# FJingxian/JanusX

Hardware: AMD Instinct MI355X
Metric: SNPs/sec full -lmm (GRM+eig+scan) (higher is better)
Workload: dtype f64 (eigendecomposition, REML and per-SNP statistics; GRM and rotation products are exact int8 / split-f16 MFMA sums merged in f64)

## Files before the change

janusx_amd/csrc/eigh.cpp:

```cpp
#include <rocblas/rocblas.h>
#include <rocsolver/rocsolver.h>

#include <stdio.h>
#include <stdlib.h>
#include <string.h>

#include <chrono>
#include <memory>
#include <mutex>
#include <vector>

#include "jx_common.h"

namespace jx {
int launch_add_diag(double *d_a, int n, int64_t ld, double ridge, hipStream_t st);
int launch_symmetrize(double *d_a, int n, hipStream_t st);
int sytrd_lower(rocblas_handle h, hipStream_t st, double *d_a, int n, double *d_d, double *d_e, double *d_tau);
int stedc_split(rocblas_handle h, hipStream_t st, int n, double *d_d, double *d_e, double *d_c, int leaf,
                std::vector<int> &h_perm, int sel_lo = 0, int sel_hi = 0);
int launch_gather_cols(const double *src, const int *d_perm, int n, double *dst, hipStream_t st);
void gather_cols_grid(int n, unsigned *gx, unsigned *gy);
int sytrd_set_dist(int rank, int world, int (*allreduce)(void *), void *user, double *staging, int64_t staging_doubles,
                   int min_n);
int ormtr_lower(hipStream_t st, const double *d_a, int n, const double *d_tau, double *d_c);
size_t sy2sb_work_doubles(int n);
int sy2sb_bandwidth();
int sy2sb_lower(hipStream_t st, double *d_a, int n, double *d_tau, double *d_ab, int ldab, double *d_work, int *d_flags,
                bool allow_shard = false);
int sy2sb_set_band_dist(int rank, int world, int (*allreduce)(void *, int64_t), void *user, double *staging,
                        int64_t staging_doubles, int min_n, int block);
int64_t sy2sb_band_staging_doubles(int n);
int sy2sb_band_dist_active(int n);
int sb2st_ldab();
int sb2st_steps(int n);
size_t sb2st_ctrl_bytes(int n);
int sb2st_chase(hipStream_t st, double *d_ab, int n, double *d_d, double *d_e, double *d_v2, double *d_tau2, int *d_ctrl);
size_t sbback_tq_doubles(int n, int ks);
int sbback_apply_q2(hipStream_t st, const double *d_v2, const double *d_tau2, int n, int ks, double *d_c, int ncols,
                    double *d_tq, hipEvent_t ev_start, hipEvent_t ev_stop);
extern float g_last_ms[24];
int ormtr_lower_off(hipStream_t st, const double *d_a, int n, int off, int nref, const double *d_tau, double *d_c, int ncols);
struct OrmtrPlan;
OrmtrPlan *ormtr_plan_new();
void ormtr_plan_free(OrmtrPlan *p);
int ormtr_prepare(hipStream_t st, const double *d_a, int n, int off, int nref, const double *d_tau, OrmtrPlan &plan);
int ormtr_apply(hipStream_t st, const OrmtrPlan &plan, double *d_c, int ncols);
int sytrd_dist_active(int n);
void sytrd_dist_rank(int *rank, int *world);
void sytrd_dist_pause(int on);
int launch_gather_cols_range(const double *src, const int *d_perm, int n, int count, double *dst, hipStream_t st);
struct EighGather {
    int (*gather)(void *) = nullptr;
    void *user = nullptr;
    int (*agree)(void *, uint64_t) = nullptr;
    void *agree_user = nullptr;
};
static EighGather g_gather;
constexpr int kRocsolverStedcMaxN = 46340;

static rocblas_handle g_handle = nullptr;
static std::mutex g_handle_mu;

static rocblas_handle get_handle() {
    std::lock_guard<std::mutex> lk(g_handle_mu);
    if (!g_handle) {
        if (rocblas_create_handle(&g_handle) != rocblas_status_success) g_handle = nullptr;
        if (g_handle) rocblas_set_atomics_mode(g_handle, rocblas_atomics_not_allowed);
    }
    return g_handle;
}
}

using namespace jx;

extern "C" int64_t jxg_eigh_dist_staging_doubles(int n) { return (int64_t)n + 32 * 16 + 2 * 64; }

// ... 108 lines not shown
        auto flag_on_any_rank = [&](int local_flag, int *any) -> int {
            *any = local_flag != 0;
            if (!dist_two) return 0;
            if (!g_gather.agree) {
                if (local_flag != 0)
                    return fail("jxg_eigh_f64: a reduction stage failed on this rank and no agreement callback is registered "
                                "(jxg_eigh_set_agree): the ranks cannot take the fallback together");
                return 0;
            }
            const int ag = g_gather.agree(g_gather.agree_user, local_flag != 0 ? 0x9e3779b97f4a7c15ull : 0ull);
            if (ag < 0) return fail("jxg_eigh_f64: the agreement callback failed");
            if (ag == 0) *any = 1;
            return 0;
        };
        std::unique_ptr<OrmtrPlan, void (*)(OrmtrPlan *)> q1_plan(nullptr, ormtr_plan_free);
        DevBuf ts_work, ts_ab, ts_tau2, ts_ctrl, ts_flags, ts_tq;
        ScratchLease ts_v2;
        const int ldab = sb2st_ldab(), ks = sb2st_steps(n);
        if (twostage) {
            if (ts_work.alloc(sizeof(double) * sy2sb_work_doubles(n))) return 1;
            if (ts_ab.alloc(sizeof(double) * (size_t)ldab * n)) return 1;
            if (ts_v2.take(4, sizeof(double) * (size_t)n * n)) return 1;
            if (ts_tau2.alloc(sizeof(double) * (size_t)n * ks)) return 1;
            if (ts_ctrl.alloc(sb2st_ctrl_bytes(n))) return 1;
            if (ts_flags.alloc(sizeof(int) * 4)) return 1;
            JX_HIP(hipMemcpyAsync(c.p, d_a, sizeof(double) * (size_t)n * n, hipMemcpyDeviceToDevice, st));
            static const bool force_single = getenv("JXGPU_DIST_EIGH_FORCE") && atoi(getenv("JXGPU_DIST_EIGH_FORCE")) != 0;
            const bool shard_band = (dist_two || force_single) && sy2sb_band_dist_active(n);
            g_last_band_sharded = shard_band ? 1 : 0;
            if (sy2sb_lower(st, d_a, n, tau.as<double>(), ts_ab.as<double>(), ldab, ts_work.as<double>(),
                            ts_flags.as<int>(), shard_band))
                return 1;
            int hf[4] = {0, 0, 0, 0};
            JX_HIP(hipMemcpyAsync(hf, ts_flags.p, sizeof(hf), hipMemcpyDeviceToHost, st));
            {
                size_t fr = 0, tot = 0;
                const size_t need = sizeof(double) * sbback_tq_doubles(n, ks);
                if (hipMemGetInfo(&fr, &tot) == hipSuccess && fr > need + ((size_t)8 << 30) && ts_tq.alloc(need)) return 1;
            }
            JX_HIP(hipStreamSynchronize(st));
            int flagged = 0;
            if (flag_on_any_rank(hf[0], &flagged)) return 1;
            if (flagged) {
                if (trace) (void)stage_done("sy2sb (flagged)");
                if (trace) fprintf(stderr, "[jxgpu eigh n=%d] band reduction flagged a panel (code %d): one-stage fallback\n", n, hf[0]);
                JX_HIP(hipMemcpyAsync(d_a, c.p, sizeof(double) * (size_t)n * n, hipMemcpyDeviceToDevice, st));
                ts_tq.release();
                twostage = false;
            }
        }
        if (twostage) {
            JX_HIP(hipEventRecord(ev[1], st));
            if (stage_done("sy2sb")) return 1;
            if (sb2st_chase(st, ts_ab.as<double>(), n, d_w, e.as<double>(), ts_v2.as<double>(), ts_tau2.as<double>(),
                            ts_ctrl.as<int>()))
                return 1;
            int habort = 0;
            JX_HIP(hipMemcpyAsync(&habort, ts_ctrl.as<int>() + n, sizeof(int), hipMemcpyDeviceToHost, st));
            JX_HIP(hipStreamSynchronize(st));
            int aborted = 0;
            if (flag_on_any_rank(habort, &aborted)) return 1;
            if (aborted) {
                if (trace) fprintf(stderr, "[jxgpu eigh n=%d] bulge chasing gave up waiting for a neighbour sweep: one-stage fallback\n", n);
                JX_HIP(hipMemcpyAsync(d_a, c.p, sizeof(double) * (size_t)n * n, hipMemcpyDeviceToDevice, st));
                ts_tq.release();
                twostage = false;
            } else {
                JX_HIP(hipEventRecord(ev[2], st));
                if (stage_done("sb2st")) return 1;
            }
        }
        if (twostage) q1_plan.reset(ormtr_plan_new());
        if (!twostage) {
            if (sytrd_lower(h, st, d_a, n, d_w, e.as<double>(), tau.as<double>())) return 1;
            if (stage_done("sytrd")) return 1;
        }
        const char *sm = getenv("JXGPU_STEDC");
        bool split = n >= 2048;
        if (sm && strcmp(sm, "rocsolver") == 0 && n <= kRocsolverStedcMaxN) split = false;
        if (sm && strcmp(sm, "split") == 0 && n >= 64) split = true;
        int leaf = getenv("JXGPU_STEDC_LEAF") ? atoi(getenv("JXGPU_STEDC_LEAF")) : 1280;
        if (leaf < 2) leaf = 2;
        if (leaf > kRocsolverStedcMaxN) leaf = kRocsolverStedcMaxN;
        std::vector<int> perm;
        rocblas_status rs = rocblas_status_success;
        bool replicas_agree = true;
        g_last_dist_agree = -1;
// ... 184 lines not shown
```

janusx_amd/csrc/k_dgemm.hip:

```cpp
#include <stdlib.h>

#include "jx_common.h"

namespace jx {

typedef double d4 __attribute__((ext_vector_type(4)));

constexpr int DG_BK = 16;
constexpr int DG_THREADS = 512;

struct DgemmArgs {
    const double *a;
    const double *b;
    double *c;
    int64_t lda, ldb, ldc;
    int m, n, k;
    double alpha, beta;
    int ta, tb;
    int symm_a;
    int lower_tiles;
    int ksplit;
    double *ws;
};

// ... 415 lines not shown
}

static int dg_reduce(hipStream_t st, const DgemmArgs &g) {
    if ((int64_t)g.m * g.n > 0xffffff00LL) return fail("dgemm: result beyond 2^32 elements (one dispatch dimension)");
    const int64_t mn = (int64_t)g.m * g.n;
    if (mn <= 16384 && g.ksplit >= 16)
        hipLaunchKernelGGL(dg_reduce_kernel<8>, dim3((unsigned)((mn + 31) / 32)), dim3(256), 0, st, g.c, g.ldc, g.m, g.n, g.beta, g.ws,
                           g.ksplit);
    else
        hipLaunchKernelGGL(dg_reduce_kernel<1>, dim3((unsigned)((mn + 255) / 256)), dim3(256), 0, st, g.c, g.ldc, g.m, g.n, g.beta, g.ws,
                           g.ksplit);
    JX_LAUNCH_CHECK();
    return 0;
}

int dgemm(hipStream_t st, bool ta, bool tb, int m, int n, int k, double alpha, const double *a, int64_t lda,
          const double *b, int64_t ldb, double beta, double *c, int64_t ldc, int ksplit, double *ws, size_t ws_doubles) {
    if (m <= 0 || n <= 0) return 0;
    DgemmArgs g{a, b, c, lda, ldb, ldc, m, n, k, alpha, beta, ta ? 1 : 0, tb ? 1 : 0, 0, 0, 1, ws};
    if (k <= 0) {
        hipLaunchKernelGGL(dg_scale_kernel, dim3((unsigned)(((int64_t)m * n + 255) / 256)), dim3(256), 0, st, c, ldc, m, n, beta);
        JX_LAUNCH_CHECK();
        return 0;
    }
    const bool small_n = n <= 64, small_m = m <= 64;
    const int bm = small_m ? 64 : 128, bn = (small_n || small_m) ? 64 : 128;
    const int tm = ceil_div(m, bm), tn = ceil_div(n, bn);
    if (ksplit <= 0) {
        const int64_t tiles = (int64_t)tm * tn;
        const int ktiles = ceil_div(k, DG_BK);
        ksplit = 1;
        if (tiles < 384) {
            ksplit = (int)((768 + tiles - 1) / tiles);
            const int maxsplit = ktiles / 8 > 0 ? ktiles / 8 : 1;
            if (ksplit > maxsplit) ksplit = maxsplit;
            if (ksplit < 1) ksplit = 1;
        }
    }
    g.ksplit = dg_fit_split(ksplit, m, n, ws ? ws_doubles : 0);
    dim3 grid(tm, tn, g.ksplit);
    int rc;
    if (bm == 128 && bn == 128) rc = dg_launch<128, 128>(g, grid, st);
    else if (bm == 128) rc = dg_launch<128, 64>(g, grid, st);
    else rc = dg_launch<64, 64>(g, grid, st);
    if (rc) return rc;
    return g.ksplit > 1 ? dg_reduce(st, g) : 0;
}

int dsymm_lower(hipStream_t st, int m, int n, double alpha, const double *a, int64_t lda, const double *b, int64_t ldb,
                double beta, double *c, int64_t ldc, double *ws, size_t ws_doubles) {
    if (m <= 0 || n <= 0) return 0;
    DgemmArgs g{a, b, c, lda, ldb, ldc, m, n, m, alpha, beta, 0, 0, 1, 0, 1, ws};
    const bool wide = n > 64;
// ... 98 lines not shown
```

janusx_amd/csrc/k_ormtr.hip:

```cpp
#include <stdlib.h>

#include <algorithm>
#include <chrono>
#include <vector>

#include "k_ozgemm.h"

namespace jx {

int dgemm(hipStream_t st, bool ta, bool tb, int m, int n, int k, double alpha, const double *a, int64_t lda, const double *b,
          int64_t ldb, double beta, double *c, int64_t ldc, int ksplit, double *ws, size_t ws_doubles);

constexpr int OT_NB = 1024;
constexpr int OT_TB = 64;

__global__ __launch_bounds__(256) void ot_extract_v_kernel(const double *__restrict__ a, int n, int jb, int nbk,
                                                          const double *__restrict__ tau, double *__restrict__ vc,
                                                          int rows, int off) {
    const int k = blockIdx.y;
    const int r = blockIdx.x * 256 + threadIdx.x;
    if (k >= nbk || r >= rows) return;
    const int j = jb + k;
    const int row = jb + off + r;
    double v = 0.0;
    if (tau[j] != 0.0) {
        if (row == j + off) v = 1.0;
        else if (row > j + off) v = a[(int64_t)j * n + row];
    }
    vc[(int64_t)k * rows + r] = v;
}

__global__ void ot_fix_m_kernel(double *__restrict__ m, int nbk, int nb, const double *__restrict__ tau, int jb) {
    const int c = blockIdx.x * blockDim.x + threadIdx.x;
    const int r = blockIdx.y;
    if (c >= nb || r >= nb) return;
    double *p = m + (int64_t)c * nb + r;
    if (r >= nbk || c >= nbk) *p = (r == c) ? 1.0 : 0.0;
    else if (r > c) *p = 0.0;
    else if (r == c) {
        const double t = tau[jb + c];
        *p = (t != 0.0) ? 1.0 / t : 1.0;
    }
}

__global__ __launch_bounds__(OT_TB) void ot_triinv_diag_kernel(const double *__restrict__ m, double *__restrict__ t, int ld) {
    __shared__ double s[OT_TB][OT_TB + 1];
    const int o = blockIdx.x * OT_TB, c = threadIdx.x;
    for (int j = 0; j < OT_TB; ++j) s[c][j] = m[(int64_t)(o + j) * ld + o + c];
    __syncthreads();
    double x[OT_TB];
#pragma unroll
    for (int i = OT_TB - 1; i >= 0; --i) {
        double acc = (i == c) ? 1.0 : 0.0;
#pragma unroll
        for (int k = i + 1; k < OT_TB; ++k) acc -= s[i][k] * x[k];
        x[i] = (i <= c) ? acc / s[i][i] : 0.0;
// ... 21 lines not shown

static int ot_round_nb(int nb) {
    int r = OT_TB;
    while (r * 2 <= nb) r *= 2;
    return r;
}

int ormtr_oz_min_n() {
    static const int v = getenv("JXGPU_OZ_MIN_N") ? atoi(getenv("JXGPU_OZ_MIN_N")) : 3000;
    return v;
}

struct OrmtrBlock {
    int jb = 0, nbk = 0, rows = 0;
    size_t o_vt = 0, o_vtt = 0;
};
struct OrmtrPlan {
    int n = 0, off = 0, nref = 0, nb = 0;
    bool use_oz = false;
    std::vector<OrmtrBlock> blocks;
    ScratchLease work;
    ScratchLease store;
};

OrmtrPlan *ormtr_plan_new() { return new OrmtrPlan(); }
void ormtr_plan_free(OrmtrPlan *p) { delete p; }

int ormtr_prepare(hipStream_t st, const double *d_a, int n, int off, int nref, const double *d_tau, OrmtrPlan &P) {
    P.n = n;
    P.off = off;
    P.nref = nref;
    P.blocks.clear();
    if (n < 2 || nref < 1) return 0;
    static const bool oz_on = !(getenv("JXGPU_ORMTR_OZ") && atoi(getenv("JXGPU_ORMTR_OZ")) == 0);
    P.use_oz = oz_on && n >= ormtr_oz_min_n();
    int nb = (getenv("JXGPU_ORMTR_NB") && atoi(getenv("JXGPU_ORMTR_NB")) > 0) ? atoi(getenv("JXGPU_ORMTR_NB"))
                                                                              : (n >= 12000 ? 2 * OT_NB : OT_NB);
    nb = ot_round_nb(std::max(nb, OT_TB));
    while (nb > OT_TB && nb / 2 >= nref) nb /= 2;
    P.nb = nb;
    const int nblocks = (nref + nb - 1) / nb;
    size_t store_bytes = 0;
    for (int b = nblocks - 1; b >= 0; --b) {
        OrmtrBlock k;
        k.jb = b * nb;
        k.nbk = (nref - k.jb < nb) ? (nref - k.jb) : nb;
        k.rows = n - k.jb - off;
        k.o_vt = store_bytes;
        store_bytes += P.use_oz ? oz_image_bytes(k.nbk, k.rows) : ((sizeof(double) * (size_t)k.rows * k.nbk + 255) & ~(size_t)255);
        k.o_vtt = store_bytes;
        store_bytes += P.use_oz ? oz_image_bytes(k.rows, k.nbk) : ((sizeof(double) * (size_t)k.rows * k.nbk + 255) & ~(size_t)255);
        P.blocks.push_back(k);
    }
    const size_t nvc = (size_t)n * nb, nmm = (size_t)nb * nb;
    const size_t ngws = std::max<size_t>(4 * nmm, (size_t)1 << 20);
    if (P.work.take(3, sizeof(double) * (2 * nvc + 2 * nmm + nmm / 4 + ngws))) return 1;
    if (P.store.take(5, store_bytes + 256)) return 1;
    double *const vc = P.work.as<double>(), *const vt = vc + nvc, *const mm = vt + nvc, *const tt = mm + nmm;
    double *const xw = tt + nmm, *const gws = xw + nmm / 4;
    char *const store = P.store.as<char>();
    for (const OrmtrBlock &k : P.blocks) {
        double *vcb = P.use_oz ? vc : reinterpret_cast<double *>(store + k.o_vt);
        double *vtb = P.use_oz ? vt : reinterpret_cast<double *>(store + k.o_vtt);
        hipLaunchKernelGGL(ot_extract_v_kernel, dim3((k.rows + 255) / 256, k.nbk), dim3(256), 0, st, d_a, n, k.jb, k.nbk, d_tau,
                           vcb, k.rows, off);
        JX_LAUNCH_CHECK();
        if (P.use_oz) {
            OzImage i_vt = oz_image_at(store + k.o_vt, k.nbk, k.rows);
            if (oz_slice(st, vcb, k.rows, 1, i_vt)) return 1;
            if (oz_mm(st, i_vt, i_vt, k.nbk, k.nbk, 1.0, 0.0, mm, nb, 1)) return 1;
        } else {
            if (dgemm(st, true, false, k.nbk, k.nbk, k.rows, 1.0, vcb, k.rows, vcb, k.rows, 0.0, mm, nb, 0, gws, ngws)) return 1;
        }
        hipLaunchKernelGGL(ot_fix_m_kernel, dim3((nb + 63) / 64, nb), dim3(64), 0, st, mm, k.nbk, nb, d_tau, k.jb);
        JX_LAUNCH_CHECK();
        if (ot_triinv_upper(st, mm, tt, nb, k.nbk, xw, gws, ngws)) return 1;
        if (dgemm(st, false, false, k.rows, k.nbk, k.nbk, 1.0, vcb, k.rows, tt, nb, 0.0, vtb, k.rows, 0, gws, ngws)) return 1;
        if (P.use_oz) {
            OzImage i_vtt = oz_image_at(store + k.o_vtt, k.rows, k.nbk);
            if (oz_slice(st, vtb, 1, k.rows, i_vtt)) return 1;
        }
    }
    return 0;
}

int ormtr_apply(hipStream_t st, const OrmtrPlan &P, double *d_c, int ncols) {
    if (P.blocks.empty() || ncols < 1) return 0;
    const int n = P.n, nb = P.nb;
    const size_t nw = (size_t)nb * ncols;
    const size_t ngws = std::max<size_t>(4 * (size_t)nb * nb, (size_t)1 << 20);
    size_t b_c = 0, b_w = 0;
    if (P.use_oz) {
        b_c = oz_image_bytes(ncols, n - P.off);
        b_w = oz_image_bytes(ncols, nb);
    }
    ScratchLease ws;
    if (ws.take(6, sizeof(double) * (nw + ngws) + b_c + b_w + 512)) return 1;
// ... 54 lines not shown
```

janusx_amd/csrc/k_ozgemm.h:

```cpp
#pragma once
#include "jx_common.h"

namespace jx {

struct OzImage {
    int8_t *q = nullptr;
    double *scale = nullptr;
    int rows = 0, k = 0, nrb = 0, nks = 0, planes = 0;
};

int oz_planes();
int oz_planes_override_get();
void oz_planes_override_set(int planes);
size_t oz_image_bytes(int rows, int k, int planes = 0);
OzImage oz_image_at(void *mem, int rows, int k, int planes = 0);
int oz_slice(hipStream_t st, const double *x, int64_t rs, int64_t cs, const OzImage &im);
int oz_mm(hipStream_t st, const OzImage &a, const OzImage &b, int m, int n, double alpha, double beta, double *c, int64_t ldc,
          int mode);
int oz_dgemm(hipStream_t st, bool ta, bool tb, int m, int n, int k, double alpha, const double *a, int64_t lda, const double *b,
             int64_t ldb, double beta, double *c, int64_t ldc, void *work, size_t work_bytes);

}
```

janusx_amd/csrc/k_ozgemm.hip:

```cpp
#include <stdlib.h>

#include "k_ozgemm.h"

namespace jx {

typedef int oz_i32x4 __attribute__((ext_vector_type(4)));
typedef int oz_i32x16 __attribute__((ext_vector_type(16)));

constexpr int OZ_TM = 128;
constexpr int OZ_BK = 32;
constexpr int OZ_PLANE = OZ_TM * OZ_BK;
constexpr int OZ_NST = 3;

static thread_local int g_oz_planes_override = 0;
int oz_planes_override_get() { return g_oz_planes_override; }
void oz_planes_override_set(int planes) { g_oz_planes_override = (planes >= 4 && planes <= 6) ? planes : 0; }
int oz_planes() {
    static const int p = [] {
        const char *e = getenv("JXGPU_OZ_PLANES");
        const int v = e ? atoi(e) : 6;
        return (v >= 4 && v <= 6) ? v : 6;
    }();
    const int o = g_oz_planes_override;
    return (o >= 4 && o <= 6) ? o : p;
// ... 238 lines not shown
            const int gn = n0 + (r & 3) + 8 * (r >> 2) + 4 * h;
            if (mok && gn < g.n) {
                double sbn = g.sb[gn];
                if (sbn == 0.0) sbn = 1.0;
                double v = (double)acc[P - 1][bj][r];
#pragma unroll
                for (int l = P - 2; l >= 0; --l) v = v * R254 + (double)acc[l][bj][r];
                v *= sam * sbn;
                double *cp = g.c + (int64_t)gn * g.ldc + gm;
                *cp = (g.beta == 0.0) ? v : fma(g.beta, *cp, v);
            }
        }
    }
}

template <int P> static int oz_slice_launch(hipStream_t st, const double *x, int64_t rs, int64_t cs, const OzImage &im) {
    int spb = 8;
    while (spb > 1 && (int64_t)im.nrb * ceil_div(im.nks, spb) < 2048) spb /= 2;
    dim3 grid((unsigned)ceil_div(im.nks, spb), (unsigned)im.nrb);
    hipLaunchKernelGGL((oz_slice_kernel<P>), grid, dim3(256), 0, st, x, rs, cs, im.rows, im.k, im.nks, spb, im.scale, im.q);
    JX_LAUNCH_CHECK();
    return 0;
}

int oz_slice(hipStream_t st, const double *x, int64_t rs, int64_t cs, const OzImage &im) {
    if (im.rows <= 0 || im.k <= 0) return 0;
    if (rs != 1 && cs != 1) return fail("oz_slice: one stride has to be 1");
    if (im.nrb > 65535) return fail("oz_slice: more than 65535 row blocks");
    JX_HIP(hipMemsetAsync(im.scale, 0, sizeof(double) * (size_t)im.nrb * OZ_TM, st));
    {
        const bool kfast = cs == 1;
        const int rgroups = kfast ? ceil_div(im.rows, 16) : ceil_div(im.rows, 256);
        int kchunk = kfast ? 2048 : 256;
        while (kchunk > 64 && (int64_t)rgroups * ceil_div(im.k, kchunk) < 2048) kchunk /= 2;
        if (rgroups > 65535) return fail("oz_slice: too many row groups");
        hipLaunchKernelGGL(oz_rowmax_kernel, dim3((unsigned)ceil_div(im.k, kchunk), (unsigned)rgroups), dim3(256), 0, st, x, rs, cs,
                           im.rows, im.k, kchunk, reinterpret_cast<unsigned long long *>(im.scale));
        JX_LAUNCH_CHECK();
    }
    switch (im.planes) {
        case 4: return oz_slice_launch<4>(st, x, rs, cs, im);
        case 5: return oz_slice_launch<5>(st, x, rs, cs, im);
        case 6: return oz_slice_launch<6>(st, x, rs, cs, im);
    }
    return fail("oz_slice: unsupported plane count");
}

template <int P> static int oz_mm_launch(hipStream_t st, const OzArgs &g) {
    static bool attr = false;
    constexpr int lds = OZ_NST * 2 * P * OZ_PLANE;
    if (!attr) {
        JX_HIP(hipFuncSetAttribute((const void *)oz_mm_kernel<P>, hipFuncAttributeMaxDynamicSharedMemorySize, lds));
        attr = true;
    }
    const int sct = ceil_div(g.tn, 4);
    const int64_t supers = (int64_t)g.srt * sct;
    const int64_t groups = (supers + 7) / 8;
    const int64_t blocks = groups * 32 * 8;
// ... 78 lines not shown
```

janusx_amd/csrc/k_sy2sb.hip:

```cpp
#include <stdlib.h>

#include <algorithm>

#include "jx_common.h"

namespace jx {

int dgemm(hipStream_t st, bool ta, bool tb, int m, int n, int k, double alpha, const double *a, int64_t lda,
          const double *b, int64_t ldb, double beta, double *c, int64_t ldc, int ksplit, double *ws, size_t ws_doubles);
int dsymm_lower(hipStream_t st, int m, int n, double alpha, const double *a, int64_t lda, const double *b, int64_t ldb,
                double beta, double *c, int64_t ldc, double *ws, size_t ws_doubles);
int dsyr2k_lower_nt(hipStream_t st, int m, int k, double alpha, const double *a, int64_t lda, const double *b, int64_t ldb,
                    double beta, double *c, int64_t ldc);

constexpr int SB = 64;
constexpr int SB_P = SB + 1;
constexpr int SB_FLAG_FAIL = 0;

static_assert(SB == 64, "the register-cyclic tiny kernels are written for SB = 64");

struct Tiny {
    double v[4][4];
};

// ... 478 lines not shown
    g_band.min_n = min_n > 0 ? min_n : 8192;
    g_band.block = block >= 2 * SB ? (block / SB) * SB : 2048;
    return 0;
}
int64_t sy2sb_band_staging_doubles(int n) {
    const int64_t b = g_band.block + 2 * SB;
    return std::max<int64_t>((int64_t)n * SB, (2 * b) * (2 * b));
}
int sy2sb_band_dist_active(int n) {
    const bool force_single = getenv("JXGPU_DIST_EIGH_FORCE") && atoi(getenv("JXGPU_DIST_EIGH_FORCE")) != 0;
    return ((g_band.world > 1 || force_single) && g_band.allreduce && n >= g_band.min_n &&
            g_band.staging_doubles >= sy2sb_band_staging_doubles(n)) ? 1 : 0;
}

int sy2sb_lower(hipStream_t st, double *d_a, int n, double *d_tau, double *d_ab, int ldab, double *d_work,
                int *d_flags, bool allow_shard) {
    const int ncol = n - SB - 1;
    JX_HIP(hipMemsetAsync(d_tau, 0, sizeof(double) * (size_t)n, st));
    JX_HIP(hipMemsetAsync(d_flags, 0, sizeof(int) * 4, st));
    if (ncol > 0) {
        double *pan[2] = {d_work, d_work + (size_t)n * 4 * SB};
        double *p = d_work + (size_t)n * 8 * SB;
        double *gq = p; p += SB * SB;
        double *gu = p; p += SB * SB;
        double *rmat = p; p += SB * SB;
        double *umat = p; p += SB * SB;
        double *rtot = p; p += SB * SB;
        double *tmat[2];
        tmat[0] = p; p += SB * SB;
        tmat[1] = p; p += SB * SB;
        double *tm = p; p += 2 * SB * SB;
// ... 136 lines not shown
                        return 1;
                } else if (for_owned(j0 + SB, nb, [&](int r0, int rl) -> int {
                               if (r0 > nb &&
                                   dgemm(st, false, true, rl, r0 - nb, 2 * SB, -1.0, v1 + r0, ld, wc + nb, ld, 1.0,
                                         a22 + r0 + (int64_t)nb * ld, ld, 1, nullptr, 0))
                                   return 1;
                               return dsyr2k_lower_nt(st, rl, 2 * SB, -1.0, v1 + r0, ld, wc + r0, ld, 1.0,
                                                      a22 + r0 + (int64_t)r0 * ld, ld);
                           })) {
                    return 1;
                }
                if (!lookahead && panel_qr(st, j0 + SB, par ^ 1, ws_main)) return 1;
            } else {
                if (dsyr2k_lower_nt(st, nt, 2 * SB, -1.0, v1, ld, wc, ld, 1.0, a22, ld)) return 1;
            }
        }
    }
    hipLaunchKernelGGL(sb_extract_band_kernel, dim3((unsigned)(((int64_t)n * ldab + 255) / 256)), dim3(256), 0, st, d_a, n,
                       d_ab, ldab);
    JX_LAUNCH_CHECK();
    return 0;
}

}
```

janusx_amd/switches.py:

```python

SWITCHES = {
    "JXGPU_OZ_PLANES": ("numerics", "6 (5 inside pipeline.eigh_from_grm(f32_consumer=True))",
                        "digit planes of the sliced int8 products of the eigensolver (4..6); 4 is NOT a product state",
                        "test_sliced_int8_gemm[5|6], test_full_size_c2/c3/c4_properties[f32_consumer], test_end_to_end_two_stage"),
    "JXGPU_EIGH_F32_PLANES": ("numerics", "5", "0 keeps 6 planes for the f32-consuming pipeline",
                              "test_full_size_c3_properties[0.0-False] (6) / [0.0-True] (5)"),
    "JXGPU_STEDC_OZ_PLANES": ("numerics", "unset (follows JXGPU_OZ_PLANES)", "planes of the divide-and-conquer merges alone", "untested"),
    "JXGPU_GRM_MISS_DIGITS": ("numerics", "3", "2 = the two-digit dense missing-call GRM of rounds 4-5 (beta off by 1e-5..1e-4 end to end)",
                              "test_end_to_end_two_stage (default); 2 is NOT a product state"),
    "JXGPU_GRM_MISS": ("numerics", "1", "0: rows with missing calls on the fp16 split kernel (f32 accumulation, like the reference)",
                       "test_grm_missing_calls_sparse_correction"),
    "JXGPU_GRM_MISS_MAX": ("numerics", "0.012", "largest missing share for the sparse correction", "test_grm_missing_calls_sparse_correction"),
    "JXGPU_GRM_MISS_DENSE_MIN": ("numerics", "0.0015", "missing share from which the dense digit form replaces the sparse correction",
                                 "test_grm_missing_calls_sparse_correction, scripts/diag_e2e_two_stage.py"),
    "JXGPU_GRM_MISS_DENSE_ROWS": ("numerics", "16384", "fewest SNPs for the dense digit form", "test_grm_missing_calls_sparse_correction"),
    "JXGPU_GRM_FP4": ("form", "0", "1: the count Gram of the 256-tile form on the fp4 matrix pipes from a nibble image (exact like the int8 kernel)",
                      "test_grm_count_gram_on_the_fp4_pipes"),
    "JXGPU_GRM_I8": ("numerics", "1", "0: exact-integer SNPs on the fp16 single-product kernel (f32 sums instead of exact i32)", "untested"),
    "JXGPU_GRM_EXACT": ("numerics", "1", "0: every SNP on the fp16 hi/lo split kernel", "untested"),
    "JXGPU_ROT_I8": ("numerics", "1", "0: design rows on the fp16 hi/lo rotation instead of the exact int8 planes",
                     "test_full_size_rotation_kernels_with_mixed_rows"),
    "JXGPU_ROT_EXACT": ("numerics", "1", "0: no integer-LUT fast path in the fp16 rotation", "untested"),
    "JXGPU_ROT_MISS_DENSE": ("numerics", "auto", "form of the missing-call term of the int8 rotation (both exact)",
                             "test_rotation_rows_with_a_few_missing_calls_take_the_exact_path"),
# ... 14 lines not shown
                   "test_eigh_two_stage_path_and_its_fallback"),
    "JXGPU_EIGH_TWOSTAGE_MIN": ("numerics", "1500", "size from which the two-stage reduction runs", "test_eigh_two_stage_path_and_its_fallback"),
    "JXGPU_STEDC": ("numerics", "own", "rocsolver: vendor divide and conquer (diagnostic)", "test_eigh_own_divide_and_conquer"),
    "JXGPU_ORMTR": ("numerics", "own", "rocsolver back-transformation (diagnostic)", "untested"),
    "JXGPU_ORMTR_OZ": ("numerics", "1", "0: Q1 on the f64 MFMA GEMM instead of the sliced int8 one", "untested"),
    "JXGPU_STEDC_OZ": ("numerics", "1", "0: merges on the f64 MFMA GEMM", "untested"),
    "JXGPU_OZ_MIN_N": ("numerics", "3000 / 750", "size from which Q1 / the merges take the sliced products", "untested"),
    "JXGPU_DIST_BACKEND": ("knob", "nccl", "collective backend of `jx` multi-rank runs", "test_cli_two_ranks_share_one_gpu"),
    "JXGPU_DIST_EIGH": ("knob", "1", "0: replicated eigendecomposition on several ranks", "test_bench_two_ranks_share_one_gpu"),
    "JXGPU_DIST_EIGH_MIN_N": ("knob", "16384", "size from which the eigensolver's stages are dealt over the ranks", "test_bench_two_ranks_share_one_gpu"),
    "JXGPU_DIST_EIGH_ONESTAGE": ("knob", "unset", "sharded one-stage reduction", "untested"),
    "JXGPU_DIST_BAND": ("knob", "1", "0: band reduction replicated", "untested"),
    "JXGPU_DIST_BAND_MIN_N": ("knob", "16384", "size from which the band reduction is sharded", "test_sharded_band_reduction_rccl_single_rank"),
    "JXGPU_DIST_BAND_BLOCK": ("test", "auto", "block rows of the sharded band reduction", "test_sharded_band_reduction_rccl_single_rank"),
    "JXGPU_DIST_DC_WINDOW": ("knob", "1", "0: top-level merge replicated", "untested"),
    "JXGPU_SYR2K_PIPE_WGS": ("knob", "7/8 of the CUs", "workgroups of the persistent rank-2k update (the rest of the CUs serve the panel chain)",
                             "test_rank_2k_update_forms_give_the_same_bits"),
    "JXGPU_SPLMM_ROUTE": ("knob", "auto", "dense | block | factor: form of K + lambda I of the sparse-GRM routes",
                          "test_splmm_block_route_matches_the_dense_route, test_splmm_giant_component_both_sides_of_the_limit"),
    "JXGPU_SPLMM_BLOCK": ("knob", "4096", "samples per diagonal block of the block route", "test_splmm_block_route_matches_the_dense_route"),
    "JXGPU_SPLMM_BLOCK_MIN_N": ("knob", "16384", "size from which the block route is taken", "untested"),
    "JXGPU_SPGRM_ACC_GB": ("knob", "auto", "HBM for the sparse-GRM builder's accumulator", "untested"),
    "JXGPU_SPECTRAL_CACHE": ("knob", "1", "0: no reuse of the last sparse GRM's decomposition", "untested"),
    **{k: ("form", "default", "kernel / launch shape of the same computation", t) for k, t in {
        "JXGPU_BC_OWNED": "test_bulge_chasing_position_owned_equals_sweep_owned", "JXGPU_SB2ST_WGS": "untested", "JXGPU_GRM_I8_TILE": "test_sparse_grm_row_panels_write_the_same_file",
        "JXGPU_GRM_TILE": "untested", "JXGPU_GRM_EXACT_BK": "untested", "JXGPU_ROT256": "untested", "JXGPU_SCAN_NOLDS": "untested",
        "JXGPU_SCAN_NOTILE": "untested", "JXGPU_SBBACK_BAL": "untested", "JXGPU_SBBACK_BAL5": "test_eigh_balanced_q2_forms",
        "JXGPU_SBBACK_BAL_MIN": "untested", "JXGPU_SBBACK_BAL_PER": "untested", "JXGPU_SBBACK_GROUPS": "untested", "JXGPU_SBBACK_NW": "untested",
        "JXGPU_SBBACK_PAIR": "untested", "JXGPU_SBBACK_SOLO": "untested", "JXGPU_STEDC_LEAF": "test_eigh_own_divide_and_conquer",
        "JXGPU_STEDC_OWNLEAF": "untested", "JXGPU_STEDC_PAR": "untested", "JXGPU_STEDC_PARMIN": "untested", "JXGPU_SY2SB_LOOKAHEAD": "untested",
# ... 35 lines not shown
```

Before: 141,000.

## Prepare Q1 reflector blocks on a side stream during the band reduction's last panels

Adds a panel hook to the band reduction. Once the trailing matrix is small, every Q1 reflector block whose columns are already final is prepared (V extraction, T-matrix inverse, VT product and int8 slicing) on a separate non-blocking stream, alongside the remaining panels. The preparation launches are capped to about three quarters of the CUs, so the rest can keep serving the panel chain. This takes part of the serial Q1 preparation off the critical path between the two-stage stages. The cost is more memory, extra events and sync, and some contention with the band reduction's own kernels.

```diff
diff --git a/janusx_amd/csrc/eigh.cpp b/janusx_amd/csrc/eigh.cpp
--- a/janusx_amd/csrc/eigh.cpp
+++ b/janusx_amd/csrc/eigh.cpp
@@ -26,7 +26,8 @@
 size_t sy2sb_work_doubles(int n);
 int sy2sb_bandwidth();
 int sy2sb_lower(hipStream_t st, double *d_a, int n, double *d_tau, double *d_ab, int ldab, double *d_work, int *d_flags,
-                bool allow_shard = false);
+                bool allow_shard = false, int (*panel_hook)(void *user, hipStream_t st, int final_cols, int nt) = nullptr,
+                void *hook_user = nullptr);
 int sy2sb_set_band_dist(int rank, int world, int (*allreduce)(void *, int64_t), void *user, double *staging,
                         int64_t staging_doubles, int min_n, int block);
 int64_t sy2sb_band_staging_doubles(int n);
@@ -43,6 +44,11 @@
 struct OrmtrPlan;
 OrmtrPlan *ormtr_plan_new();
 void ormtr_plan_free(OrmtrPlan *p);
+size_t ormtr_plan_bytes(int n, int off, int nref);
+int ormtr_plan_begin(OrmtrPlan &plan, int n, int off, int nref);
+int ormtr_plan_blocks(const OrmtrPlan &plan);
+int ormtr_plan_block_end(const OrmtrPlan &plan, int b);
+int ormtr_prepare_block(hipStream_t st, OrmtrPlan &plan, int b, const double *d_a, const double *d_tau, int max_wgs);
 int ormtr_prepare(hipStream_t st, const double *d_a, int n, int off, int nref, const double *d_tau, OrmtrPlan &plan);
 int ormtr_apply(hipStream_t st, const OrmtrPlan &plan, double *d_c, int ncols);
 int sytrd_dist_active(int n);
@@ -60,6 +66,29 @@
 
 static rocblas_handle g_handle = nullptr;
 static std::mutex g_handle_mu;
+
+struct Q1Tail {
+    OrmtrPlan *plan = nullptr;
+    const double *a = nullptr, *tau = nullptr;
+    int nt_max = 0, max_wgs = 0, next_block = 0;
+    hipStream_t prep = nullptr;
+    hipEvent_t ev_final = nullptr, ev_done = nullptr;
+};
+static int q1_tail_hook(void *user, hipStream_t st, int final_cols, int nt) {
+    Q1Tail &q = *static_cast<Q1Tail *>(user);
+    if (nt > q.nt_max) return 0;
+    bool ordered = false;
+    while (q.next_block + 1 < ormtr_plan_blocks(*q.plan) && ormtr_plan_block_end(*q.plan, q.next_block) <= final_cols) {
+        if (!ordered) {
+            JX_HIP(hipEventRecord(q.ev_final, st));
+            JX_HIP(hipStreamWaitEvent(q.prep, q.ev_final, 0));
+            ordered = true;
+        }
+        if (ormtr_prepare_block(q.prep, *q.plan, q.next_block, q.a, q.tau, q.max_wgs)) return 1;
+        ++q.next_block;
+    }
+    return 0;
+}
 
 static rocblas_handle get_handle() {
     std::lock_guard<std::mutex> lk(g_handle_mu);
@@ -198,6 +227,7 @@
             return 0;
         };
         std::unique_ptr<OrmtrPlan, void (*)(OrmtrPlan *)> q1_plan(nullptr, ormtr_plan_free);
+        Q1Tail q1_tail;
         DevBuf ts_work, ts_ab, ts_tau2, ts_ctrl, ts_flags, ts_tq;
         ScratchLease ts_v2;
         const int ldab = sb2st_ldab(), ks = sb2st_steps(n);
@@ -212,9 +242,44 @@
             static const bool force_single = getenv("JXGPU_DIST_EIGH_FORCE") && atoi(getenv("JXGPU_DIST_EIGH_FORCE")) != 0;
             const bool shard_band = (dist_two || force_single) && sy2sb_band_dist_active(n);
             g_last_band_sharded = shard_band ? 1 : 0;
+            const int q1_tail_nt = getenv("JXGPU_Q1_TAIL_NT") ? atoi(getenv("JXGPU_Q1_TAIL_NT")) : 8192;
+            const int q1_nref = n - sy2sb_bandwidth() - 1;
+            if (q1_tail_nt > 0 && !dist_two && !force_single && q1_nref > 0) {
+                size_t fr = 0, tot = 0;
+                const size_t need = ormtr_plan_bytes(n, sy2sb_bandwidth(), q1_nref) + sizeof(double) * sbback_tq_doubles(n, ks);
+                if (hipMemGetInfo(&fr, &tot) == hipSuccess && fr > need + ((size_t)8 << 30)) {
+                    static hipStream_t prep = nullptr;
+                    static hipEvent_t ev_prep[2] = {nullptr, nullptr};
+                    static int tail_wgs = 0;
+                    if (!prep) {
+                        JX_HIP(hipEventCreateWithFlags(&ev_prep[0], hipEventDisableTiming));
+                        JX_HIP(hipEventCreateWithFlags(&ev_prep[1], hipEventDisableTiming));
+                        int dev = 0, cus = 0;
+                        JX_HIP(hipGetDevice(&dev));
+                        JX_HIP(hipDeviceGetAttribute(&cus, hipDeviceAttributeMultiprocessorCount, dev));
+                        tail_wgs = getenv("JXGPU_Q1_TAIL_WGS") ? atoi(getenv("JXGPU_Q1_TAIL_WGS")) : cus * 3 / 4;
+                        if (tail_wgs < 16) tail_wgs = 16;
+                        JX_HIP(hipStreamCreateWithFlags(&prep, hipStreamNonBlocking));
+                    }
+                    q1_plan.reset(ormtr_plan_new());
+                    if (ormtr_plan_begin(*q1_plan, n, sy2sb_bandwidth(), q1_nref)) return 1;
+                    q1_tail.plan = q1_plan.get();
+                    q1_tail.a = d_a;
+                    q1_tail.tau = tau.as<double>();
+                    q1_tail.nt_max = q1_tail_nt;
+                    q1_tail.max_wgs = tail_wgs;
+                    q1_tail.prep = prep;
+                    q1_tail.ev_final = ev_prep[0];
+                    q1_tail.ev_done = ev_prep[1];
+                }
+            }
             if (sy2sb_lower(st, d_a, n, tau.as<double>(), ts_ab.as<double>(), ldab, ts_work.as<double>(),
-                            ts_flags.as<int>(), shard_band))
+                            ts_flags.as<int>(), shard_band, q1_tail.plan ? q1_tail_hook : nullptr, &q1_tail))
                 return 1;
+            if (q1_tail.plan && q1_tail.next_block > 0) {
+                JX_HIP(hipEventRecord(q1_tail.ev_done, q1_tail.prep));
+                JX_HIP(hipStreamWaitEvent(st, q1_tail.ev_done, 0));
+            }
             int hf[4] = {0, 0, 0, 0};
             JX_HIP(hipMemcpyAsync(hf, ts_flags.p, sizeof(hf), hipMemcpyDeviceToHost, st));
             {
@@ -228,6 +293,9 @@
             if (flagged) {
                 if (trace) (void)stage_done("sy2sb (flagged)");
                 if (trace) fprintf(stderr, "[jxgpu eigh n=%d] band reduction flagged a panel (code %d): one-stage fallback\n", n, hf[0]);
+                if (q1_tail.plan) JX_HIP(hipStreamSynchronize(q1_tail.prep));
+                q1_tail.plan = nullptr;
+                q1_plan.reset();
                 JX_HIP(hipMemcpyAsync(d_a, c.p, sizeof(double) * (size_t)n * n, hipMemcpyDeviceToDevice, st));
                 ts_tq.release();
                 twostage = false;
@@ -246,6 +314,9 @@
             if (flag_on_any_rank(habort, &aborted)) return 1;
             if (aborted) {
                 if (trace) fprintf(stderr, "[jxgpu eigh n=%d] bulge chasing gave up waiting for a neighbour sweep: one-stage fallback\n", n);
+                if (q1_tail.plan) JX_HIP(hipStreamSynchronize(q1_tail.prep));
+                q1_tail.plan = nullptr;
+                q1_plan.reset();
                 JX_HIP(hipMemcpyAsync(d_a, c.p, sizeof(double) * (size_t)n * n, hipMemcpyDeviceToDevice, st));
                 ts_tq.release();
                 twostage = false;
@@ -254,7 +325,7 @@
                 if (stage_done("sb2st")) return 1;
             }
         }
-        if (twostage) q1_plan.reset(ormtr_plan_new());
+        if (twostage && !q1_plan) q1_plan.reset(ormtr_plan_new());
         if (!twostage) {
             if (sytrd_lower(h, st, d_a, n, d_w, e.as<double>(), tau.as<double>())) return 1;
             if (stage_done("sytrd")) return 1;
diff --git a/janusx_amd/csrc/k_dgemm.hip b/janusx_amd/csrc/k_dgemm.hip
--- a/janusx_amd/csrc/k_dgemm.hip
+++ b/janusx_amd/csrc/k_dgemm.hip
@@ -453,6 +453,22 @@
     return 0;
 }
 
+int dgemm_auto_split(int m, int n, int k, size_t ws_doubles) {
+    if (m <= 0 || n <= 0 || k <= 0) return 1;
+    const bool small_n = n <= 64, small_m = m <= 64;
+    const int bm = small_m ? 64 : 128, bn = (small_n || small_m) ? 64 : 128;
+    const int64_t tiles = (int64_t)ceil_div(m, bm) * ceil_div(n, bn);
+    const int ktiles = ceil_div(k, DG_BK);
+    int ksplit = 1;
+    if (tiles < 384) {
+        ksplit = (int)((768 + tiles - 1) / tiles);
+        const int maxsplit = ktiles / 8 > 0 ? ktiles / 8 : 1;
+        if (ksplit > maxsplit) ksplit = maxsplit;
+        if (ksplit < 1) ksplit = 1;
+    }
+    return dg_fit_split(ksplit, m, n, ws_doubles);
+}
+
 int dgemm(hipStream_t st, bool ta, bool tb, int m, int n, int k, double alpha, const double *a, int64_t lda,
           const double *b, int64_t ldb, double beta, double *c, int64_t ldc, int ksplit, double *ws, size_t ws_doubles) {
     if (m <= 0 || n <= 0) return 0;
@@ -465,17 +481,7 @@
     const bool small_n = n <= 64, small_m = m <= 64;
     const int bm = small_m ? 64 : 128, bn = (small_n || small_m) ? 64 : 128;
     const int tm = ceil_div(m, bm), tn = ceil_div(n, bn);
-    if (ksplit <= 0) {
-        const int64_t tiles = (int64_t)tm * tn;
-        const int ktiles = ceil_div(k, DG_BK);
-        ksplit = 1;
-        if (tiles < 384) {
-            ksplit = (int)((768 + tiles - 1) / tiles);
-            const int maxsplit = ktiles / 8 > 0 ? ktiles / 8 : 1;
-            if (ksplit > maxsplit) ksplit = maxsplit;
-            if (ksplit < 1) ksplit = 1;
-        }
-    }
+    if (ksplit <= 0) ksplit = dgemm_auto_split(m, n, k, ws ? ws_doubles : 0);
     g.ksplit = dg_fit_split(ksplit, m, n, ws ? ws_doubles : 0);
     dim3 grid(tm, tn, g.ksplit);
     int rc;
diff --git a/janusx_amd/csrc/k_ormtr.hip b/janusx_amd/csrc/k_ormtr.hip
--- a/janusx_amd/csrc/k_ormtr.hip
+++ b/janusx_amd/csrc/k_ormtr.hip
@@ -10,6 +10,7 @@
 
 int dgemm(hipStream_t st, bool ta, bool tb, int m, int n, int k, double alpha, const double *a, int64_t lda, const double *b,
           int64_t ldb, double beta, double *c, int64_t ldc, int ksplit, double *ws, size_t ws_doubles);
+int dgemm_auto_split(int m, int n, int k, size_t ws_doubles);
 
 constexpr int OT_NB = 1024;
 constexpr int OT_TB = 64;
@@ -17,29 +18,31 @@
 __global__ __launch_bounds__(256) void ot_extract_v_kernel(const double *__restrict__ a, int n, int jb, int nbk,
                                                           const double *__restrict__ tau, double *__restrict__ vc,
                                                           int rows, int off) {
-    const int k = blockIdx.y;
     const int r = blockIdx.x * 256 + threadIdx.x;
-    if (k >= nbk || r >= rows) return;
-    const int j = jb + k;
+    if (r >= rows) return;
     const int row = jb + off + r;
-    double v = 0.0;
-    if (tau[j] != 0.0) {
-        if (row == j + off) v = 1.0;
-        else if (row > j + off) v = a[(int64_t)j * n + row];
-    }
-    vc[(int64_t)k * rows + r] = v;
+    for (int k = blockIdx.y; k < nbk; k += gridDim.y) {
+        const int j = jb + k;
+        double v = 0.0;
+        if (tau[j] != 0.0) {
+            if (row == j + off) v = 1.0;
+            else if (row > j + off) v = a[(int64_t)j * n + row];
+        }
+        vc[(int64_t)k * rows + r] = v;
+    }
 }
 
 __global__ void ot_fix_m_kernel(double *__restrict__ m, int nbk, int nb, const double *__restrict__ tau, int jb) {
     const int c = blockIdx.x * blockDim.x + threadIdx.x;
-    const int r = blockIdx.y;
-    if (c >= nb || r >= nb) return;
-    double *p = m + (int64_t)c * nb + r;
-    if (r >= nbk || c >= nbk) *p = (r == c) ? 1.0 : 0.0;
-    else if (r > c) *p = 0.0;
-    else if (r == c) {
-        const double t = tau[jb + c];
-        *p = (t != 0.0) ? 1.0 / t : 1.0;
+    if (c >= nb) return;
+    for (int r = blockIdx.y; r < nb; r += gridDim.y) {
+        double *p = m + (int64_t)c * nb + r;
+        if (r >= nbk || c >= nbk) *p = (r == c) ? 1.0 : 0.0;
+        else if (r > c) *p = 0.0;
+        else if (r == c) {
+            const double t = tau[jb + c];
+            *p = (t != 0.0) ? 1.0 / t : 1.0;
+        }
     }
 }
 
@@ -91,10 +94,13 @@
 struct OrmtrBlock {
     int jb = 0, nbk = 0, rows = 0;
     size_t o_vt = 0, o_vtt = 0;
+    bool prepared = false;
 };
 struct OrmtrPlan {
     int n = 0, off = 0, nref = 0, nb = 0;
     bool use_oz = false;
+    bool begun = false;
+    size_t work_doubles = 0, store_bytes = 0;
     std::vector<OrmtrBlock> blocks;
     ScratchLease work;
     ScratchLease store;
@@ -103,12 +109,13 @@
 OrmtrPlan *ormtr_plan_new() { return new OrmtrPlan(); }
 void ormtr_plan_free(OrmtrPlan *p) { delete p; }
 
-int ormtr_prepare(hipStream_t st, const double *d_a, int n, int off, int nref, const double *d_tau, OrmtrPlan &P) {
+static void ot_plan_layout(OrmtrPlan &P, int n, int off, int nref) {
     P.n = n;
     P.off = off;
     P.nref = nref;
     P.blocks.clear();
-    if (n < 2 || nref < 1) return 0;
+    P.work_doubles = P.store_bytes = 0;
+    if (n < 2 || nref < 1) return;
     static const bool oz_on = !(getenv("JXGPU_ORMTR_OZ") && atoi(getenv("JXGPU_ORMTR_OZ")) == 0);
     P.use_oz = oz_on && n >= ormtr_oz_min_n();
     int nb = (getenv("JXGPU_ORMTR_NB") && atoi(getenv("JXGPU_ORMTR_NB")) > 0) ? atoi(getenv("JXGPU_ORMTR_NB"))
@@ -131,33 +138,93 @@
     }
     const size_t nvc = (size_t)n * nb, nmm = (size_t)nb * nb;
     const size_t ngws = std::max<size_t>(4 * nmm, (size_t)1 << 20);
-    if (P.work.take(3, sizeof(double) * (2 * nvc + 2 * nmm + nmm / 4 + ngws))) return 1;
-    if (P.store.take(5, store_bytes + 256)) return 1;
+    P.work_doubles = 2 * nvc + 2 * nmm + nmm / 4 + ngws;
+    P.store_bytes = store_bytes + 256;
+}
+
+size_t ormtr_plan_bytes(int n, int off, int nref) {
+    OrmtrPlan P;
+    ot_plan_layout(P, n, off, nref);
+    return sizeof(double) * P.work_doubles + P.store_bytes;
+}
+
+int ormtr_plan_begin(OrmtrPlan &P, int n, int off, int nref) {
+    if (P.begun) return fail("ormtr_plan_begin: the plan is in use");
+    ot_plan_layout(P, n, off, nref);
+    P.begun = true;
+    if (P.blocks.empty()) return 0;
+    if (P.work.take(3, sizeof(double) * P.work_doubles)) return 1;
+    if (P.store.take(5, P.store_bytes)) return 1;
+    return 0;
+}
+
+int ormtr_plan_blocks(const OrmtrPlan &P) { return (int)P.blocks.size(); }
+int ormtr_plan_block_end(const OrmtrPlan &P, int b) {
+    const OrmtrBlock &k = P.blocks[P.blocks.size() - 1 - (size_t)b];
+    return k.jb + k.nbk;
+}
+bool ormtr_plan_block_prepared(const OrmtrPlan &P, int b) { return P.blocks[P.blocks.size() - 1 - (size_t)b].prepared; }
+
+int ormtr_prepare_block(hipStream_t st, OrmtrPlan &P, int b, const double *d_a, const double *d_tau, int max_wgs) {
+    if (!P.begun || b < 0 || b >= (int)P.blocks.size()) return fail("ormtr_prepare_block: no such block");
+    OrmtrBlock &k = P.blocks[P.blocks.size() - 1 - (size_t)b];
+    if (k.prepared) return 0;
+    const int n = P.n, nb = P.nb, off = P.off;
+    const size_t nvc = (size_t)n * nb, nmm = (size_t)nb * nb;
+    const size_t ngws = std::max<size_t>(4 * nmm, (size_t)1 << 20);
     double *const vc = P.work.as<double>(), *const vt = vc + nvc, *const mm = vt + nvc, *const tt = mm + nmm;
     double *const xw = tt + nmm, *const gws = xw + nmm / 4;
     char *const store = P.store.as<char>();
-    for (const OrmtrBlock &k : P.blocks) {
-        double *vcb = P.use_oz ? vc : reinterpret_cast<double *>(store + k.o_vt);
-        double *vtb = P.use_oz ? vt : reinterpret_cast<double *>(store + k.o_vtt);
-        hipLaunchKernelGGL(ot_extract_v_kernel, dim3((k.rows + 255) / 256, k.nbk), dim3(256), 0, st, d_a, n, k.jb, k.nbk, d_tau,
-                           vcb, k.rows, off);
+    double *vcb = P.use_oz ? vc : reinterpret_cast<double *>(store + k.o_vt);
+    double *vtb = P.use_oz ? vt : reinterpret_cast<double *>(store + k.o_vtt);
+    const int cap = max_wgs > 0 ? max_wgs : 0;
+    {
+        const int gx = (k.rows + 255) / 256;
+        const int gy = cap ? std::max(1, std::min(k.nbk, cap / gx)) : k.nbk;
+        hipLaunchKernelGGL(ot_extract_v_kernel, dim3(gx, gy), dim3(256), 0, st, d_a, n, k.jb, k.nbk, d_tau, vcb, k.rows, off);
         JX_LAUNCH_CHECK();
-        if (P.use_oz) {
-            OzImage i_vt = oz_image_at(store + k.o_vt, k.nbk, k.rows);
-            if (oz_slice(st, vcb, k.rows, 1, i_vt)) return 1;
-            if (oz_mm(st, i_vt, i_vt, k.nbk, k.nbk, 1.0, 0.0, mm, nb, 1)) return 1;
-        } else {
-            if (dgemm(st, true, false, k.nbk, k.nbk, k.rows, 1.0, vcb, k.rows, vcb, k.rows, 0.0, mm, nb, 0, gws, ngws)) return 1;
-        }
-        hipLaunchKernelGGL(ot_fix_m_kernel, dim3((nb + 63) / 64, nb), dim3(64), 0, st, mm, k.nbk, nb, d_tau, k.jb);
+    }
+    if (P.use_oz) {
+        OzImage i_vt = oz_image_at(store + k.o_vt, k.nbk, k.rows);
+        if (oz_slice(st, vcb, k.rows, 1, i_vt, cap)) return 1;
+        if (oz_mm(st, i_vt, i_vt, k.nbk, k.nbk, 1.0, 0.0, mm, nb, 1)) return 1;
+    } else {
+        if (dgemm(st, true, false, k.nbk, k.nbk, k.rows, 1.0, vcb, k.rows, vcb, k.rows, 0.0, mm, nb, 0, gws, ngws)) return 1;
+    }
+    {
+        const int gx = (nb + 63) / 64;
+        const int gy = cap ? std::max(1, std::min(nb, cap / gx)) : nb;
+        hipLaunchKernelGGL(ot_fix_m_kernel, dim3(gx, gy), dim3(64), 0, st, mm, k.nbk, nb, d_tau, k.jb);
         JX_LAUNCH_CHECK();
-        if (ot_triinv_upper(st, mm, tt, nb, k.nbk, xw, gws, ngws)) return 1;
+    }
+    if (ot_triinv_upper(st, mm, tt, nb, k.nbk, xw, gws, ngws)) return 1;
+    const int tn = (k.nbk + 127) / 128, tm = (k.rows + 127) / 128;
+    const int ks = dgemm_auto_split(k.rows, k.nbk, k.nbk, ngws);
+    if (!cap || tm == 1 || (int64_t)tm * tn * ks <= cap) {
         if (dgemm(st, false, false, k.rows, k.nbk, k.nbk, 1.0, vcb, k.rows, tt, nb, 0.0, vtb, k.rows, 0, gws, ngws)) return 1;
-        if (P.use_oz) {
-            OzImage i_vtt = oz_image_at(store + k.o_vtt, k.rows, k.nbk);
-            if (oz_slice(st, vtb, 1, k.rows, i_vtt)) return 1;
-        }
-    }
+    } else {
+        const int per = std::max(1, cap / (tn * ks));
+        for (int t0 = 0; t0 < tm;) {
+            int t1 = std::min(tm, t0 + per);
+            if (t1 == tm - 1 && k.rows - t1 * 128 <= 64) t1 = (t1 - t0 > 1) ? t1 - 1 : tm;
+            const int r0 = t0 * 128, rl = std::min(k.rows, t1 * 128) - r0;
+            if (dgemm(st, false, false, rl, k.nbk, k.nbk, 1.0, vcb + r0, k.rows, tt, nb, 0.0, vtb + r0, k.rows, ks, gws, ngws)) return 1;
+            t0 = t1;
+        }
+    }
+    if (P.use_oz) {
+        OzImage i_vtt = oz_image_at(store + k.o_vtt, k.rows, k.nbk);
+        if (oz_slice(st, vtb, 1, k.rows, i_vtt, cap)) return 1;
+    }
+    k.prepared = true;
+    return 0;
+}
+
+int ormtr_prepare(hipStream_t st, const double *d_a, int n, int off, int nref, const double *d_tau, OrmtrPlan &P) {
+    if (!P.begun && ormtr_plan_begin(P, n, off, nref)) return 1;
+    if (P.n != n || P.off != off || P.nref != nref) return fail("ormtr_prepare: the plan was begun for another problem");
+    for (int b = (int)P.blocks.size() - 1; b >= 0; --b)
+        if (ormtr_prepare_block(st, P, b, d_a, d_tau, 0)) return 1;
     return 0;
 }
 
diff --git a/janusx_amd/csrc/k_ozgemm.h b/janusx_amd/csrc/k_ozgemm.h
--- a/janusx_amd/csrc/k_ozgemm.h
+++ b/janusx_amd/csrc/k_ozgemm.h
@@ -14,7 +14,7 @@
 void oz_planes_override_set(int planes);
 size_t oz_image_bytes(int rows, int k, int planes = 0);
 OzImage oz_image_at(void *mem, int rows, int k, int planes = 0);
-int oz_slice(hipStream_t st, const double *x, int64_t rs, int64_t cs, const OzImage &im);
+int oz_slice(hipStream_t st, const double *x, int64_t rs, int64_t cs, const OzImage &im, int max_wgs = 0);
 int oz_mm(hipStream_t st, const OzImage &a, const OzImage &b, int m, int n, double alpha, double beta, double *c, int64_t ldc,
           int mode);
 int oz_dgemm(hipStream_t st, bool ta, bool tb, int m, int n, int k, double alpha, const double *a, int64_t lda, const double *b,
diff --git a/janusx_amd/csrc/k_ozgemm.hip b/janusx_amd/csrc/k_ozgemm.hip
--- a/janusx_amd/csrc/k_ozgemm.hip
+++ b/janusx_amd/csrc/k_ozgemm.hip
@@ -276,34 +276,61 @@
     }
 }
 
-template <int P> static int oz_slice_launch(hipStream_t st, const double *x, int64_t rs, int64_t cs, const OzImage &im) {
+template <int P> static int oz_slice_launch(hipStream_t st, const double *x, int64_t rs, int64_t cs, const OzImage &im, int max_wgs) {
     int spb = 8;
-    while (spb > 1 && (int64_t)im.nrb * ceil_div(im.nks, spb) < 2048) spb /= 2;
-    dim3 grid((unsigned)ceil_div(im.nks, spb), (unsigned)im.nrb);
-    hipLaunchKernelGGL((oz_slice_kernel<P>), grid, dim3(256), 0, st, x, rs, cs, im.rows, im.k, im.nks, spb, im.scale, im.q);
-    JX_LAUNCH_CHECK();
+    if (max_wgs <= 0) {
+        while (spb > 1 && (int64_t)im.nrb * ceil_div(im.nks, spb) < 2048) spb /= 2;
+        dim3 grid((unsigned)ceil_div(im.nks, spb), (unsigned)im.nrb);
+        hipLaunchKernelGGL((oz_slice_kernel<P>), grid, dim3(256), 0, st, x, rs, cs, im.rows, im.k, im.nks, spb, im.scale, im.q);
+        JX_LAUNCH_CHECK();
+        return 0;
+    }
+    while (ceil_div(im.nks, spb) > max_wgs) spb *= 2;
+    const int gx = ceil_div(im.nks, spb), per = std::max(1, max_wgs / gx);
+    for (int rb0 = 0; rb0 < im.nrb; rb0 += per) {
+        const int nrbc = std::min(per, im.nrb - rb0);
+        const int rows = std::min(im.rows - rb0 * OZ_TM, nrbc * OZ_TM);
+        hipLaunchKernelGGL((oz_slice_kernel<P>), dim3((unsigned)gx, (unsigned)nrbc), dim3(256), 0, st, x + (int64_t)rb0 * OZ_TM * rs, rs,
+                           cs, rows, im.k, im.nks, spb, im.scale + (size_t)rb0 * OZ_TM,
+                           im.q + (int64_t)rb0 * im.nks * (P * OZ_PLANE));
+        JX_LAUNCH_CHECK();
+    }
     return 0;
 }
 
-int oz_slice(hipStream_t st, const double *x, int64_t rs, int64_t cs, const OzImage &im) {
+int oz_slice(hipStream_t st, const double *x, int64_t rs, int64_t cs, const OzImage &im, int max_wgs) {
     if (im.rows <= 0 || im.k <= 0) return 0;
     if (rs != 1 && cs != 1) return fail("oz_slice: one stride has to be 1");
     if (im.nrb > 65535) return fail("oz_slice: more than 65535 row blocks");
     JX_HIP(hipMemsetAsync(im.scale, 0, sizeof(double) * (size_t)im.nrb * OZ_TM, st));
     {
         const bool kfast = cs == 1;
-        const int rgroups = kfast ? ceil_div(im.rows, 16) : ceil_div(im.rows, 256);
+        const int rpg = kfast ? 16 : 256;
+        const int rgroups = ceil_div(im.rows, rpg);
         int kchunk = kfast ? 2048 : 256;
-        while (kchunk > 64 && (int64_t)rgroups * ceil_div(im.k, kchunk) < 2048) kchunk /= 2;
         if (rgroups > 65535) return fail("oz_slice: too many row groups");
-        hipLaunchKernelGGL(oz_rowmax_kernel, dim3((unsigned)ceil_div(im.k, kchunk), (unsigned)rgroups), dim3(256), 0, st, x, rs, cs,
-                           im.rows, im.k, kchunk, reinterpret_cast<unsigned long long *>(im.scale));
-        JX_LAUNCH_CHECK();
+        unsigned long long *const sc = reinterpret_cast<unsigned long long *>(im.scale);
+        if (max_wgs <= 0) {
+            while (kchunk > 64 && (int64_t)rgroups * ceil_div(im.k, kchunk) < 2048) kchunk /= 2;
+            hipLaunchKernelGGL(oz_rowmax_kernel, dim3((unsigned)ceil_div(im.k, kchunk), (unsigned)rgroups), dim3(256), 0, st, x, rs, cs,
+                               im.rows, im.k, kchunk, sc);
+            JX_LAUNCH_CHECK();
+        } else {
+            while (ceil_div(im.k, kchunk) > max_wgs) kchunk *= 2;
+            const int gx = ceil_div(im.k, kchunk), per = std::max(1, max_wgs / gx);
+            for (int g0 = 0; g0 < rgroups; g0 += per) {
+                const int ng = std::min(per, rgroups - g0);
+                const int rows = std::min(im.rows - g0 * rpg, ng * rpg);
+                hipLaunchKernelGGL(oz_rowmax_kernel, dim3((unsigned)gx, (unsigned)ng), dim3(256), 0, st, x + (int64_t)g0 * rpg * rs, rs,
+                                   cs, rows, im.k, kchunk, sc + (size_t)g0 * rpg);
+                JX_LAUNCH_CHECK();
+            }
+        }
     }
     switch (im.planes) {
-        case 4: return oz_slice_launch<4>(st, x, rs, cs, im);
-        case 5: return oz_slice_launch<5>(st, x, rs, cs, im);
-        case 6: return oz_slice_launch<6>(st, x, rs, cs, im);
+        case 4: return oz_slice_launch<4>(st, x, rs, cs, im, max_wgs);
+        case 5: return oz_slice_launch<5>(st, x, rs, cs, im, max_wgs);
+        case 6: return oz_slice_launch<6>(st, x, rs, cs, im, max_wgs);
     }
     return fail("oz_slice: unsupported plane count");
 }
diff --git a/janusx_amd/csrc/k_sy2sb.hip b/janusx_amd/csrc/k_sy2sb.hip
--- a/janusx_amd/csrc/k_sy2sb.hip
+++ b/janusx_amd/csrc/k_sy2sb.hip
@@ -516,7 +516,8 @@
 }
 
 int sy2sb_lower(hipStream_t st, double *d_a, int n, double *d_tau, double *d_ab, int ldab, double *d_work,
-                int *d_flags, bool allow_shard) {
+                int *d_flags, bool allow_shard, int (*panel_hook)(void *user, hipStream_t st, int final_cols, int nt),
+                void *hook_user) {
     const int ncol = n - SB - 1;
     JX_HIP(hipMemsetAsync(d_tau, 0, sizeof(double) * (size_t)n, st));
     JX_HIP(hipMemsetAsync(d_flags, 0, sizeof(int) * 4, st));
@@ -683,6 +684,7 @@
             } else {
                 if (dsyr2k_lower_nt(st, nt, 2 * SB, -1.0, v1, ld, wc, ld, 1.0, a22, ld)) return 1;
             }
+            if (panel_hook && panel_hook(hook_user, st, j0 + pw, nt)) return 1;
         }
     }
     hipLaunchKernelGGL(sb_extract_band_kernel, dim3((unsigned)(((int64_t)n * ldab + 255) / 256)), dim3(256), 0, st, d_a, n,
diff --git a/janusx_amd/switches.py b/janusx_amd/switches.py
--- a/janusx_amd/switches.py
+++ b/janusx_amd/switches.py
@@ -52,6 +52,11 @@
     "JXGPU_DIST_BAND_MIN_N": ("knob", "16384", "size from which the band reduction is sharded", "test_sharded_band_reduction_rccl_single_rank"),
     "JXGPU_DIST_BAND_BLOCK": ("test", "auto", "block rows of the sharded band reduction", "test_sharded_band_reduction_rccl_single_rank"),
     "JXGPU_DIST_DC_WINDOW": ("knob", "1", "0: top-level merge replicated", "untested"),
+    "JXGPU_Q1_TAIL_NT": ("knob", "8192", "trailing size of the band reduction from which complete Q1 reflector blocks are prepared beside "
+                         "its last panels (same bits); 0: all of them in line in front of the Q1 products",
+                         "test_q1_blocks_prepared_beside_the_band_reduction_give_the_same_bits"),
+    "JXGPU_Q1_TAIL_WGS": ("knob", "3/4 of the CUs", "largest launch of that preparation in workgroups (the rest of the CUs serve the panel chain)",
+                          "test_q1_blocks_prepared_beside_the_band_reduction_give_the_same_bits (default)"),
     "JXGPU_SYR2K_PIPE_WGS": ("knob", "7/8 of the CUs", "workgroups of the persistent rank-2k update (the rest of the CUs serve the panel chain)",
                              "test_rank_2k_update_forms_give_the_same_bits"),
     "JXGPU_SPLMM_ROUTE": ("knob", "auto", "dense | block | factor: form of K + lambda I of the sparse-GRM routes",
```

After: 142,600 (median of 6 runs). 1.1% higher.
